# Borda/pyImSegm

Hardware: AMD Instinct MI355X
Metric: Mpixels/s end-to-end SLIC+fts+GC, 2048x2048 RGB; % HBM roofline (higher is better)
Workload: dtype f64; 1 GPU; single 2048x2048 RGB uint8 per GPU, SLIC(sp_size=46, K=2025, 10 sweeps) + colour mean/std/energy + 3-class alpha-expansion GC (gc_regul=2.0, edge=model), pre-fitted GMM, host numpy in -> segm int32 in host numpy (BASELINE configs[1]); bench_config=2, images_per_launch_chain=1, images_in_flight_per_gpu=4, hardware_queues=4, input_memory=pageable numpy, input_ring=default (one rank: measured in round 4), parallelism=images sharded over 1 GPU(s), 4 in flight per GPU (one HIP stream each)

## Files before the change

pyimsegm_amd/_hip.py:

```python
import ctypes as C
import functools
import os
import threading

import numpy as np

_HERE = os.path.dirname(os.path.abspath(__file__))
LIB_PATH = os.environ.get('IMSEGM_HIP_LIBRARY') or os.path.join(_HERE, 'libimsegm_hip.so')

U8, F64, F32 = 0, 1, 2
PROFILE_GROUPS = {
    'slic_assign': 0,
    'slic': 1,
    'connectivity': 2,
    'color_stats': 3,
    'graph': 4,
    'graphcut': 5,
    'gather': 6,
    'slic_preprocess': 7,
    'terms': 8,
    'texture': 9,
}


# ... 1066 lines not shown
        out = np.empty((count.value, 4), dtype=np.float32 if code.value == F32 else np.float64)
        _check(lib.imsegm_volume_get_centroids(self._h, _ptr(out), C.byref(code), C.byref(count)))
        return out

    def label_cc(self):
        n_out = C.c_int(0)
        _check(load_library().imsegm_volume_label_cc(self._h, C.byref(n_out)))
        self.n_labels = n_out.value
        return self.n_labels

    def gray_stats(self, mean=True, energy=True, var=True):
        k = self.n_labels
        m = np.empty(k, dtype=np.float64) if mean else None
        e = np.empty(k, dtype=np.float64) if energy else None
        v = np.empty(k, dtype=np.float64) if var else None
        _check(load_library().imsegm_volume_gray_stats(self._h, _ptr(m), _ptr(e), _ptr(v)))
        return m, e, v

    def graph(self):
        k = self.n_labels
        cap = max(64, 8 * k)
        centres = np.empty((k, 3), dtype=np.float64)
        present = np.empty(k, dtype=np.uint8)
        while True:
            edges = np.empty((cap, 2), dtype=np.int32)
            ne = C.c_int(0)
            _check(load_library().imsegm_volume_graph(self._h, _ptr(edges), cap, C.byref(ne), _ptr(centres),
                                                      _ptr(present)))
            if ne.value <= cap:
                return edges[:ne.value], centres, present.astype(bool)
            cap = ne.value

    def _unsupported(self, *args, **kwargs):
        raise HipError('not available for volumes')

    get_lab = color_stats = run_color = _unsupported

    def lm_prepare(self, sigma=150.):
        taps = gaussian_taps(sigma)
        _check(load_library().imsegm_image2d_lm_prepare(self._h, _ptr(taps), len(taps) - 1, None))
        return self

    def response_stats(self, mul, div, mean=True, energy=True, var=True):
        k = self.n_labels
        m = np.empty(k, dtype=np.float64) if mean else None
        e = np.empty(k, dtype=np.float64) if energy else None
        v = np.empty(k, dtype=np.float64) if var else None
        _check(load_library().imsegm_image2d_response_stats(self._h, float(mul), float(div), _ptr(m), _ptr(e), _ptr(v)))
        return m, e, v

    def response_median(self, mul, div):
        out = np.empty(self.n_labels, dtype=np.float64)
        _check(load_library().imsegm_image2d_response_median(self._h, float(mul), float(div), _ptr(out)))
        return out

    def response_mean_gradient(self, mul, div):
        out = np.empty(self.n_labels, dtype=np.float64)
        _check(load_library().imsegm_image2d_response_mean_gradient(self._h, float(mul), float(div), _ptr(out)))
        return out

    def get_response(self):
        out = np.empty(self.shape, dtype=np.float64)
        _check(load_library().imsegm_image2d_get_response(self._h, _ptr(out)))
        return out


class Batch2D(object):

    def __init__(self, max_images, height, width, ctx=None):
        self.ctx = ctx or default_context()
        self.shape = (int(height), int(width))
        self.max_images = int(max_images)
        self._h = _vp()
        self.n_labels = []
        self.n_images = 0
        _check(load_library().imsegm_batch2d_create(self.ctx._h, self.max_images, self.shape[0], self.shape[1], C.byref(self._h)))
        self.ctx.users += 1

    def close(self):
        if self._h and self.ctx is not None:
            self.ctx.users -= 1
            if self.ctx._h and self.ctx.pid == os.getpid():
                load_library().imsegm_batch2d_destroy(self._h)
        self._h = None

    def __del__(self):
        try:
            self.close()
        except Exception:
            pass

    def run_color(self, images, n_segments, compactness, gmm, pairwise, edge_type='model', feature_flags=(True, True, True),
                  sigma=1., normalize=2, max_iter=10, start_label=0, edge_cost=1., use_graphcut=True, classes=None, to_host=True,
                  pinned=True, out=None):
        images = [np.ascontiguousarray(im) for im in images]
        if not 0 < len(images) <= self.max_images:
            raise ValueError('between 1 and %d images per batch' % self.max_images)
        dtype = images[0].dtype
        if dtype not in _DTYPES or any(im.shape != self.shape + (3, ) or im.dtype != dtype for im in images):
            raise ValueError('expected images of shape %r + (3,) and one dtype of uint8 / float32 / float64' % (self.shape, ))
        code = EDGE_TYPES.get(edge_type)
        if code is None:
            raise ValueError('edge type %r is not evaluated on the device' % (edge_type, ))
        pairwise = np.ascontiguousarray(pairwise, dtype=np.float64)
        nc = gmm.n_classes
        if pairwise.shape != (nc, nc):
            raise ValueError('pairwise cost must be %d x %d' % (nc, nc))
        cl = None if classes is None else np.ascontiguousarray(classes, dtype=np.int32)
        taps = gaussian_taps(sigma)
        r = -1 if taps is None else len(taps) - 1
        n = len(images)
        src = (_vp * n)(*[im.ctypes.data for im in images])
        segm, dst = None, None
        if to_host:
            if out is not None:
                segm = list(out)
                if len(segm) != n or any(a.shape != self.shape or a.dtype != np.int32 or not a.flags['C_CONTIGUOUS'] for a in segm):
                    raise ValueError('out: one C-contiguous int32 array of the image size per image')
            else:
                alloc = pinned_empty if pinned else np.empty
                segm = [alloc(self.shape, np.int32) for _ in range(n)]
            dst = (_vp * n)(*[a.ctypes.data for a in segm])
        mask = (1 if feature_flags[0] else 0) | (2 if feature_flags[1] else 0) | (4 if feature_flags[2] else 0)
        counts = (C.c_int * n)()
        _check(load_library().imsegm_batch2d_run_color(
            self._h, n, src, _DTYPES[dtype], int(normalize), int(n_segments), float(compactness), _ptr(taps), r, int(max_iter),
            int(start_label), mask, C.byref(gmm.params), nc, _ptr(pairwise), code, float(edge_cost), int(bool(use_graphcut)), _ptr(cl),
            dst, counts))
        self.n_labels = list(counts)
        self.n_images = n
        self._feature_columns = 3 * bin(mask).count('1')
        self._uploaded = images
        return segm

    def _device_array(self, image, which):
        ptr = _vp()
        _check(load_library().imsegm_batch2d_device_ptr(self._h, int(image), which, C.byref(ptr)))
        return DeviceArray(ptr.value, self.shape, '<i4', self)

    def segm_device_array(self, image):
        return self._device_array(image, 1)

    def labels_device_array(self, image):
        return self._device_array(image, 0)

    def get_features(self, image):
        ptr = _vp()
        _check(load_library().imsegm_batch2d_device_ptr(self._h, int(image), 2, C.byref(ptr)))
        out = np.empty((self.n_labels[image], self._feature_columns), dtype=np.float64)
        if out.size:
            self.ctx.copy(out.ctypes.data, ptr.value, out.nbytes, synchronize=True)
        return out

    def get_labels(self, image):
        arr = self.labels_device_array(image)
        out = np.empty(self.shape, dtype=np.int32)
        self.ctx.copy(out.ctypes.data, arr.__cuda_array_interface__['data'][0], out.nbytes, synchronize=True)
        return out.astype(np.int64)


class DeviceArray(object):

    def __init__(self, ptr, shape, typestr, owner):
        self.owner = owner
        self.__cuda_array_interface__ = {'shape': tuple(shape), 'typestr': typestr, 'data': (int(ptr), False),
                                         'version': 2, 'strides': None}


def gc_grid_fallbacks():
    return int(load_library().imsegm_debug_gc_grid_fallbacks())


def exclusive_scan(values):
    values = np.ascontiguousarray(values, dtype=np.int32)
    out, total = np.empty_like(values), C.c_int(0)
    _check(load_library().imsegm_debug_exclusive_scan(values.ctypes.data, values.size, out.ctypes.data, C.byref(total)))
    return out, total.value


def slic_sweep_runs():
    a, b = C.c_long(0), C.c_long(0)
    _check(load_library().imsegm_debug_slic_sweep_runs(C.byref(a), C.byref(b)))
    return a.value, b.value


def assign_sweeps_per_launch(max_iter=10):
    persistent, fallback = slic_sweep_runs()
    return max_iter - 1 if (persistent > 0 and fallback == 0) else 1


def _device_array(sess, which, shape, typestr):
    ptr = _vp()
    _check(load_library().imsegm_image2d_device_ptr(sess._h, which, C.byref(ptr)))
    sess.ctx.synchronize()
    return DeviceArray(ptr.value, shape, typestr, sess)


def segm_device_array(sess):
    return _device_array(sess, 1, sess.shape, '<i4')


def cut_general_graph(edges, edge_weights, unary_cost, pairwise_cost, n_iter=-1, algorithm='expansion',
                      return_energy=False, ctx=None):
    if algorithm != 'expansion':
        raise NotImplementedError('only algorithm="expansion" is implemented on the HIP path')
    ctx = ctx or default_context()
    edges = np.ascontiguousarray(np.asarray(edges).reshape(-1, 2), dtype=np.int32)
    ew = np.ascontiguousarray(edge_weights, dtype=np.float64)
    un = np.ascontiguousarray(unary_cost, dtype=np.float64)
    pw = np.ascontiguousarray(pairwise_cost, dtype=np.float64)
    if un.ndim != 2 or pw.shape != (un.shape[1], un.shape[1]) or len(ew) != len(edges):
        raise ValueError('shape mismatch among edges %r, weights %r, unary %r, pairwise %r' %
                         (edges.shape, ew.shape, un.shape, pw.shape))
    labels = np.empty(un.shape[0], dtype=np.int32)
    energy = C.c_int64(0)
    _check(load_library().imsegm_cut_general_graph(ctx._h, _ptr(edges), len(edges), _ptr(ew), _ptr(un), un.shape[0],
                                                   un.shape[1], _ptr(pw), int(n_iter), _ptr(labels), C.byref(energy)))
    return (labels, energy.value) if return_energy else labels


def cut_grid_graph(unary_cost, pairwise_cost, cost_v, cost_h, n_iter=-1, algorithm='expansion', ctx=None):
    unary_cost = np.asarray(unary_cost, dtype=np.float64)
    if unary_cost.ndim != 3:
        raise ValueError('unary_cost must be height x width x labels')
    height, width, n_labels = unary_cost.shape
    cost_v, cost_h = np.asarray(cost_v, dtype=np.float64), np.asarray(cost_h, dtype=np.float64)
    if cost_v.shape != (height - 1, width) or cost_h.shape != (height, width - 1):
        raise ValueError('cost_v / cost_h do not match the grid %d x %d' % (height, width))
    index = np.arange(height * width, dtype=np.int32).reshape(height, width)
    edges = np.concatenate([np.stack([index[:-1].ravel(), index[1:].ravel()], axis=1),
                            np.stack([index[:, :-1].ravel(), index[:, 1:].ravel()], axis=1)], axis=0)
    weights = np.concatenate([cost_v.ravel(), cost_h.ravel()])
    return cut_general_graph(edges, weights, unary_cost.reshape(height * width, n_labels), pairwise_cost, n_iter=n_iter,
                             algorithm=algorithm, ctx=ctx)


def assume_bg_on_boundary(work, strips, bg_label, ctx=None):
    found = C.c_int(0)
    ctx = ctx or default_context()
    _check(load_library().imsegm_assume_bg_on_boundary(ctx._h, _ptr(work), work.shape[0], work.shape[1], _ptr(strips), int(bg_label),
                                                       C.byref(found)))
    return found.value


def label_hist2d(segm, windows, struc_elem, nb_labels, ctx=None):
    ctx = ctx or default_context()
    segm = np.ascontiguousarray(segm, dtype=np.int16)
    selem = np.ascontiguousarray(struc_elem, dtype=np.int16)
    windows = np.ascontiguousarray(windows, dtype=np.int32).reshape(-1, 6)
    out = np.zeros((len(windows), int(nb_labels)), dtype=np.uint32)
    _check(load_library().imsegm_label_hist2d(ctx._h, _ptr(segm), segm.shape[0], segm.shape[1], _ptr(windows), len(windows),
                                              _ptr(selem), selem.shape[0], selem.shape[1], int(nb_labels), _ptr(out)))
    return out


BOUNDARY_THICK, BOUNDARY_CONTOUR, BOUNDARY_CONTOUR_BORDER = 0, 1, 2


def boundary_mask(labels, mode, label=0, ctx=None):
    ctx = ctx or default_context()
    out = np.empty(labels.shape, dtype=np.uint8)
    _check(load_library().imsegm_boundary_mask(ctx._h, _ptr(labels), labels.shape[0], labels.shape[1], int(mode), int(label), _ptr(out)))
    return out


def distance_map(labels, mode, label=0, ctx=None):
    ctx = ctx or default_context()
    out = np.empty(labels.shape, dtype=np.float64)
    _check(load_library().imsegm_distance_map(ctx._h, _ptr(labels), labels.shape[0], labels.shape[1], int(mode), int(label), _ptr(out)))
    return out


def _boundary_distances(call, shape):
    capacity = int(shape[0]) * int(shape[1])
    points, dist, count = np.empty((capacity, 2), dtype=np.int32), np.empty(capacity, dtype=np.float64), C.c_int(0)
    _check(call(_ptr(points), _ptr(dist), capacity, C.byref(count)))
    return points[:count.value], dist[:count.value].copy()


def boundary_distances(segm_ref, segm, ctx=None):
    ctx = ctx or default_context()
    lib = load_library()
    return _boundary_distances(lambda *out: lib.imsegm_boundary_distances(ctx._h, _ptr(segm_ref), _ptr(segm), segm.shape[0],
                                                                          segm.shape[1], *out), segm.shape)


def labels_overlap(seg1, seg2, n_labels1, n_labels2, ctx=None):
    ctx = ctx or default_context()
    out = np.empty((int(n_labels1), int(n_labels2)), dtype=np.int64)
    _check(load_library().imsegm_labels_overlap(ctx._h, _ptr(seg1), _ptr(seg2), seg1.size, int(n_labels1), int(n_labels2), _ptr(out)))
    return out


def ellipse_ransac(point_offsets, points, params, success, trial_egg, points_all, point_value, residual_threshold,
                   with_residuals=False, ctx=None):
    ctx = ctx or default_context()
    point_offsets = np.ascontiguousarray(point_offsets, dtype=np.int32).ravel()
    points = np.ascontiguousarray(points, dtype=np.float64).reshape(-1, 2)
    params = np.ascontiguousarray(params, dtype=np.float64).reshape(-1, 5)
    success = np.ascontiguousarray(success, dtype=np.uint8).ravel()
    trial_egg = np.ascontiguousarray(trial_egg, dtype=np.int32).ravel()
    points_all = np.ascontiguousarray(points_all, dtype=np.float64).reshape(-1, 2)
    point_value = np.ascontiguousarray(point_value, dtype=np.float64).ravel()
    n_eggs, n_trials = len(point_offsets) - 1, len(params)
    if len(success) != n_trials or len(trial_egg) != n_trials or len(point_value) != len(points_all):
        raise ValueError('ellipse_ransac: one success flag and one egg per trial, one value per centre')
# ... 180 lines not shown
```

pyimsegm_amd/csrc/batch.hip:

```cpp
#include "backhalf.h"

#include <string>

struct imsegm_batch2d {
    imsegm_ctx *ctx = nullptr;
    int B = 0, H = 0, W = 0;
    size_t n = 0;
    DevBuf arena;
    size_t slice = 0;
    std::vector<unsigned char> key;
    int *fail_host = nullptr;
    void *pinned = nullptr;
    size_t pinned_cap = 0;
    int last_n = 0;
    std::vector<int> n_labels;
};

namespace {

using namespace imsegm;

inline size_t al256(size_t v) { return (v + 255) & ~(size_t)255; }

struct Layout {
    size_t img, lab, nearest, labels, conn_i32, conn_i32_bytes, conn_u8, small, cent, tiles, feat, featK, seg, segm_out, total;
    ParamBlock par;
    TermsScratch scr;
    size_t d_edges, d_as, d_at, d_ar, d_ea, d_deg, d_dlow, d_es, d_wp, d_cacc, d_bitmap, d_cent, d_present;
    int Kb, Ecap;
};

Layout make_layout(int H, int W, size_t elem, int K_grid, size_t n_tiles, long min_size, int C, int F, int Fm, int n_in)
{
    Layout L;
    memset(&L, 0, sizeof(L));
    const size_t n = (size_t)H * W;
    L.Kb = (int)std::min<size_t>(n / (size_t)std::max<long>(min_size, 1) + 2, n + 2);
    L.Ecap = 3 * L.Kb + 64;
    size_t o = 0;
    auto take = [&](size_t bytes) { size_t at = o; o += al256(bytes); return at; };
    L.small = take(4096);
    L.img = take(n * 3 * elem + 64);
    L.lab = take(3 * n * sizeof(double));
    L.nearest = take(n * 4);
    L.labels = take(n * 4);
    L.conn_i32_bytes = conn_i32_bytes(n, H, W);
    L.conn_i32 = take(L.conn_i32_bytes);
    L.conn_u8 = take(2 * n + 64);
    L.cent = take(slic_cent_bytes(K_grid));
    L.tiles = take(slic_tiles_bytes(n_tiles, n));
    const size_t Kb = (size_t)L.Kb, E = (size_t)L.Ecap, words = (size_t)cdiv(L.Kb, 32);
    L.feat = take(stats_scratch_bytes(Kb));
    L.featK = take(Kb * (size_t)std::max(F, 1) * 8 + 64);
    L.segm_out = take(n * 4);
    L.par = param_block(C, Fm, 0, n_in);
    L.scr = terms_scratch(L.par, L.Kb, C, F, L.Ecap, false, n_in ? Fm : 0);
    size_t q = L.scr.end;
    auto sub = [&](size_t bytes) { size_t at = q; q += al64(bytes); return at; };
    L.d_edges = sub(E * 8);
    L.d_as = sub((Kb + 1) * 4);
    L.d_at = sub(E * 8);
    L.d_ar = sub(E * 8);
    L.d_ea = sub(E * 8);
    L.d_deg = sub(Kb * 4);
    L.d_dlow = sub(Kb * 4);
    L.d_es = sub(Kb * 4);
    L.d_wp = sub(Kb * words * 4);
    L.d_cacc = sub(Kb * 4 * 8);
    L.d_bitmap = sub(Kb * words * 4);
    L.d_cent = sub(Kb * 3 * 8);
    L.d_present = sub(Kb);
    L.seg = take(q + 256);
    L.total = al256(o);
    return L;
}

int batch_pinned(imsegm_batch2d *bt, size_t bytes)
{
    if (bytes <= bt->pinned_cap) return 0;
    if (bt->pinned) (void)hipHostFree(bt->pinned);
    bt->pinned = nullptr;
    bt->pinned_cap = 0;
    HIP_TRY(hipHostMalloc(&bt->pinned, bytes + 4096, hipHostMallocDefault));
    bt->pinned_cap = bytes + 4096;
    return 0;
}

}

extern "C" {

int imsegm_batch2d_create(imsegm_ctx *ctx, int max_images, int height, int width, imsegm_batch2d **batch_out)
{
    if (bind(ctx)) return -1;
    if (!batch_out || max_images < 1 || max_images > 1024 || height <= 0 || width <= 0 || (long)height * width > 0x3fffffffL) {
        set_error("batch2d: 1..1024 images of a valid size");
        return -1;
    }
    imsegm_batch2d *bt = new imsegm_batch2d();
    bt->ctx = ctx;
    bt->B = max_images;
    bt->H = height;
    bt->W = width;
    bt->n = (size_t)height * width;
    bt->n_labels.assign(max_images, 0);
    *batch_out = bt;
    return 0;
}

void imsegm_batch2d_destroy(imsegm_batch2d *bt)
{
    if (!bt) return;
    (void)hipSetDevice(bt->ctx->device);
    (void)hipStreamSynchronize(bt->ctx->stream);
    bt->arena.release();
    if (bt->fail_host) (void)hipHostFree(bt->fail_host);
    if (bt->pinned) (void)hipHostFree(bt->pinned);
    delete bt;
}

int imsegm_batch2d_device_ptr(imsegm_batch2d *bt, int image, int which, void **ptr_out)
{
    if (!bt || bind(bt->ctx)) return -1;
    if (!ptr_out || image < 0 || image >= bt->last_n || bt->key.size() != sizeof(Layout)) {
        set_error("batch2d_device_ptr: no such image in the last batch");
        return -1;
    }
    Layout L;
    memcpy(&L, bt->key.data(), sizeof(L));
    unsigned char *base = bt->arena.as<unsigned char>() + (size_t)image * bt->slice;
    if (which == 0) *ptr_out = base + L.labels;
    else if (which == 1) *ptr_out = base + L.segm_out;
    else if (which == 2) *ptr_out = base + L.featK;
    else {
        set_error("batch2d_device_ptr: which = 0 (label map), 1 (segmentation) or 2 (feature table)");
        return -1;
    }
    return 0;
}

int imsegm_batch2d_run_color(imsegm_batch2d *bt, int n_images, const void *const *host_pixels, int dtype, int minmax_normalize,
                             int n_segments, double compactness, const double *taps, int radius, int max_iter, int start_label,
                             int feature_mask, const imsegm_gmm *gmm, int n_classes, const double *pairwise, int edge_type,
                             double edge_cost, int use_graphcut, const int32_t *classes_lut, int32_t *const *segm_out,
                             int *n_labels_out)
{
    if (!bt || bind(bt->ctx)) return -1;
    imsegm_ctx *ctx = bt->ctx;
    hipStream_t st = ctx->stream;
    const int H = bt->H, W = bt->W, C = n_classes;
    const size_t n = bt->n;
    if (n_images < 1 || n_images > bt->B || !host_pixels) {
        set_error("batch2d_run_color: between 1 and the batch's capacity of images");
        return -1;
    }
    const size_t es = dtype == IMSEGM_U8 ? 1 : dtype == IMSEGM_F32 ? 4 : dtype == IMSEGM_F64 ? 8 : 0;
    if (!es) {
        set_error("unsupported dtype");
        return -1;
    }
    if (!(compactness > 0) || n_segments < 1 || max_iter < 1 || (start_label != 0 && start_label != 1)) {
        set_error("slic: n_segments, compactness and max_iter must be positive, start_label 0 or 1");
        return -1;
    }
    if (feature_mask < 1 || feature_mask > 7 || !gmm || C < 1 || C > 16 || !pairwise) {
        set_error("batch2d_run_color: colour features (mask 1..7), a device class model, 1..16 classes and a pairwise matrix are required");
        return -1;
    }
    BackHalf bh;
    if (decode_edge_type(edge_type, &bh.edge_code, &bh.spatial_norm)) return -1;
    const int F = color_feature_columns(feature_mask);
    if (check_gmm(gmm, F, C)) return -1;
    if (check_pairwise(pairwise, C)) return -1;
    Taps tz, ty, tx;
    if (fill_taps(tz, taps, radius) || fill_taps(ty, taps, radius) || fill_taps(tx, taps, radius)) return -1;
    if (radius > 8 || knobs().pre_3pass) {
        set_error("batch2d_run_color: blur radius above 8 (sigma > 2) takes the single-image path");
        return -1;
    }

    SlicState s;
    SlicGeometry geo;
    if (slic_geometry(H, W, n_segments, compactness, minmax_normalize, 0, 0, s, geo)) return -1;
    const int K = geo.K;
    const double segment_size = (double)n / (double)K;
    const long min_size = (long)(0.5 * segment_size), max_size = (long)(3.0 * segment_size);
    if (min_size < 1) {
        set_error("batch2d_run_color: superpixels of under two pixels take the single-image path");
        return -1;
    }
    const Layout L = make_layout(H, W, es, K, geo.n_tiles, min_size, C, F, gmm->n_features, gmm->n_inputs);
    const size_t slice = L.total;
    const size_t stage_row = al256(std::max<size_t>(L.par.bytes, 256));
    const size_t arena_bytes = slice * bt->B + stage_row * bt->B + 4096;
    const bool same = bt->key.size() == sizeof(L) && !memcmp(bt->key.data(), &L, sizeof(L)) && bt->slice == slice && bt->arena.cap >= arena_bytes;
    if (!same) {
        HIP_TRY(hipStreamSynchronize(st));
        if (bt->arena.ensure(arena_bytes)) return -1;
        HIP_TRY(hipMemsetAsync(bt->arena.p, 0, bt->arena.cap, st));
        bt->slice = slice;
        bt->key.assign(reinterpret_cast<const unsigned char *>(&L), reinterpret_cast<const unsigned char *>(&L) + sizeof(L));
    }
    if (!bt->fail_host) HIP_TRY(hipHostMalloc((void **)&bt->fail_host, 64, hipHostMallocDefault));
    unsigned char *base = bt->arena.as<unsigned char>();
    unsigned char *stage_dev = base + slice * bt->B;
    ZBatch zb;
    zb.nz = n_images;
    zb.zs = slice;
    bt->last_n = n_images;

    bool all_pinned = true;
    for (int b = 0; b < n_images; ++b) {
        if (!host_pixels[b]) {
            set_error("batch2d_run_color: null image");
            return -1;
        }
        HIP_TRY(hipMemcpyAsync(base + (size_t)b * slice + L.img, host_pixels[b], n * 3 * es, hipMemcpyHostToDevice, st));
        all_pinned = all_pinned && is_pinned(host_pixels[b]);
    }
    if (!all_pinned) HIP_TRY(hipStreamSynchronize(st));

    unsigned long long *keys = reinterpret_cast<unsigned long long *>(base + L.small);
    double *minmax = reinterpret_cast<double *>(keys + 2);
    double *premax = minmax + 2;
    double *lab = reinterpret_cast<double *>(base + L.lab);
    int32_t *nearest = reinterpret_cast<int32_t *>(base + L.nearest), *labels = reinterpret_cast<int32_t *>(base + L.labels);
    const int sp_all = ctx->begin(PG_SLIC);
    const int sp_pre = ctx->begin(PG_PRE);
    if (launch_minmax(base + L.img, dtype, n * 3, keys, minmax, st, premax, zb)) return -1;
    if (launch_preprocess_color2d(base + L.img, dtype, H, W, minmax_normalize, minmax, tz, ty, tx, 1.0 / compactness, lab, nullptr, premax,
                                  st, true, zb))
        return -1;
    ctx->end(sp_pre);
    slic_place_state(s, geo, base + L.cent, base + L.tiles, premax, bt->fail_host);
    const ProfHook hook = ctx->hook();
    bool fused_update = false;
    if (launch_slic_iterations(s, lab, nullptr, nearest, max_iter, 0, hook, st, &fused_update, zb)) return -1;

    ConnWork w = conn_work_from(reinterpret_cast<int32_t *>(base + L.conn_i32), L.conn_i32_bytes, base + L.conn_u8, n);
    std::vector<int> &nl = bt->n_labels;
    for (int attempt = 0; attempt < 2; ++attempt) {
        if (attempt == 1) {
            slic_sweep_note_fallback();
            SlicState plain = s;
            plain.done = nullptr;
            if (launch_slic_iterations(plain, lab, nullptr, nearest, max_iter, 0, hook, st, nullptr, zb)) return -1;
        }
        const int spc = ctx->begin(PG_CONN);
        if (launch_enforce_connectivity_batch(nearest, H, W, min_size, max_size, start_label, w, labels, nl.data(), st, zb,
                                              reinterpret_cast<int32_t *>(stage_dev)))
            return -1;
        ctx->end(spc);
        if (!fused_update || *bt->fail_host == 0) break;
        fused_update = false;
    }
    for (int b = 0; b < n_images; ++b) {
        if (nl[b] >= 0) continue;
        unsigned char *sb = base + (size_t)b * slice;
        ConnWork wb = conn_work_from(reinterpret_cast<int32_t *>(sb + L.conn_i32), L.conn_i32_bytes, sb + L.conn_u8, n);
        int got = 0;
        if (launch_enforce_connectivity(reinterpret_cast<int32_t *>(sb + L.nearest), 1, H, W, min_size, max_size, start_label, wb,
                                        reinterpret_cast<int32_t *>(sb + L.labels), &got, st))
            return -1;
        nl[b] = got;
    }
    ctx->end(sp_all);
    int K_cap = 1;
    for (int b = 0; b < n_images; ++b) {
        if (nl[b] > L.Kb) {
            set_error("batch2d_run_color: more labels than the bound the buffers were sized for");
            return -1;
        }
        K_cap = std::max(K_cap, nl[b]);
        if (n_labels_out) n_labels_out[b] = nl[b];
    }
    const int words = cdiv(K_cap, 32);
    const int Ecap = std::min(L.Ecap, 3 * K_cap + 64);

    {
        const StatsScratch ss = stats_scratch_at(base + L.feat, L.Kb);
        const double *mm_dev = nullptr;
        if (dtype != IMSEGM_U8) {
            if (launch_minmax(base + L.img, dtype, n * 3, keys, minmax, st, nullptr, zb)) return -1;
            mm_dev = minmax;
        }
        const int sps = ctx->begin(PG_STATS);
        if (launch_color_stats(base + L.img, dtype, labels, H, W, K_cap, 255.0, (feature_mask & 2) != 0, ss.acc, ss.mean, ss.energy, ss.var,
                               ss.mean32, st, 0, 0, 1.0, 1.0, -1, nullptr, zb, mm_dev))
// ... 59 lines not shown
```

pyimsegm_amd/csrc/slic_pre.hip:

```cpp
#include "slic.h"
#include <hip/hip_ext.h>
#include <atomic>
#include <cstdio>


namespace imsegm {

__device__ __forceinline__ unsigned long long f64_key(double x)
{
    long long b = __double_as_longlong(x);
    return b < 0 ? ~(unsigned long long)b : ((unsigned long long)b | 0x8000000000000000ULL);
}
__host__ __device__ __forceinline__ double key_f64(unsigned long long k)
{
    unsigned long long b = (k & 0x8000000000000000ULL) ? (k & 0x7fffffffffffffffULL) : ~k;
    union { unsigned long long u; double d; } cv;
    cv.u = b;
    return cv.d;
}

__device__ __forceinline__ void block_minmax_commit(double mn, double mx, unsigned long long *keys, double *out2, double *also_zero)
{
    __shared__ double smn[4], smx[4];
    mn = wave_min_f64(mn);
// ... 103 lines not shown
    if (tz.r < 0) return v;
    double tmp = v * tz.w[0];
    for (int j = tz.r; j >= 1; --j) tmp += (v + v) * tz.w[j];
    return tmp;
}

template <int MAXR>
__device__ __forceinline__ double zblur_point_unrolled(double v, const Taps &tz)
{
    if (tz.r < 0) return v;
    double tmp = v * tz.w[0];
    const double vv = v + v;
#pragma unroll
    for (int j = MAXR; j >= 1; --j)
        if (j <= tz.r) tmp += vv * tz.w[j];
    return tmp;
}

__global__ void __launch_bounds__(256)
k_pre_lab_u8(const uint8_t *__restrict__ img, int n, int normalize, const double *__restrict__ minmax,
             Taps tz, double *__restrict__ out)
{
    __shared__ double lut[256];
    {
        int v = threadIdx.x;
        double x;
        const bool norm = normalize == 1 || (normalize == 2 && (minmax[0] != 0.0 || minmax[1] != 1.0));
        if (norm) {
            double vmin = minmax[0], range = minmax[1] - minmax[0];
            x = (double)(uint8_t)(v - (int)vmin) / range;
        } else {
            x = (double)v * (1.0 / 255);
        }
        lut[v] = (x > 0.04045) ? det_pow24((x + 0.055) / 1.055) : x / 12.92;
    }
    __syncthreads();
    int p = blockIdx.x * blockDim.x + threadIdx.x;
    if (p >= n) return;
    double lin0 = lut[img[3 * (size_t)p + 0]], lin1 = lut[img[3 * (size_t)p + 1]], lin2 = lut[img[3 * (size_t)p + 2]];
    double X = lin0 * 0.412453 + lin1 * 0.357580 + lin2 * 0.180423;
    double Y = lin0 * 0.212671 + lin1 * 0.715160 + lin2 * 0.072169;
    double Z = lin0 * 0.019334 + lin1 * 0.119193 + lin2 * 0.950227;
    double f[3] = { X / 0.95047, Y / 1.0, Z / 1.08883 };
#pragma unroll
    for (int c = 0; c < 3; ++c) {
        double t = f[c];
        f[c] = (t > 0.008856) ? det_cbrt(t) : 7.787 * t + 16.0 / 116.0;
    }
    double L = (116.0 * f[1]) - 16.0;
    double A = 500.0 * (f[0] - f[1]);
    double B = 200.0 * (f[1] - f[2]);
    out[p] = zblur_point(L, tz);
    out[(size_t)n + p] = zblur_point(A, tz);
    out[2 * (size_t)n + p] = zblur_point(B, tz);
}

template <typename T>
__global__ void __launch_bounds__(256)
k_pre_lab_f(const T *__restrict__ img, int n, int normalize, const double *__restrict__ minmax, Taps tz,
            double *__restrict__ out)
{
    int p = blockIdx.x * blockDim.x + threadIdx.x;
    if (p >= n) return;
    double rgb[3];
    const bool norm = normalize == 1 || (normalize == 2 && (minmax[0] != 0.0 || minmax[1] != 1.0));
#pragma unroll
    for (int c = 0; c < 3; ++c) {
        double v = (double)img[3 * (size_t)p + c];
        if (norm) v = (v - minmax[0]) / (minmax[1] - minmax[0]);
        rgb[c] = v;
    }
    double L, A, B;
    rgb2lab_px(rgb[0], rgb[1], rgb[2], L, A, B);
    out[p] = zblur_point(L, tz);
    out[(size_t)n + p] = zblur_point(A, tz);
    out[2 * (size_t)n + p] = zblur_point(B, tz);
}

__device__ __forceinline__ void block_absmax_to(double v, double *out)
{
    __shared__ unsigned long long wave_max[16];
    unsigned long long b = (unsigned long long)__double_as_longlong(v);
#pragma unroll
    for (int off = 32; off > 0; off >>= 1) {
        unsigned long long o = __shfl_xor(b, off, 64);
        b = o > b ? o : b;
    }
    const int wave = threadIdx.x >> 6, nw = (blockDim.x + 63) >> 6;
    if ((threadIdx.x & 63) == 0) wave_max[wave] = b;
    __syncthreads();
    if (threadIdx.x == 0) {
        for (int i = 1; i < nw; ++i) b = wave_max[i] > b ? wave_max[i] : b;
        if (b) atomicMax(reinterpret_cast<unsigned long long *>(out), b);
    }
}

__global__ void __launch_bounds__(256) k_absmax_f64(const double *__restrict__ src, size_t n, double *out)
{
    double m = 0.0;
    for (size_t i = (size_t)blockIdx.x * 256 + threadIdx.x; i < n; i += (size_t)gridDim.x * 256) m = fmax(m, fabs(src[i]));
    block_absmax_to(m, out);
}

int launch_absmax_f64(const double *src, size_t n, double *out_dev, hipStream_t st)
{
    HIP_TRY(hipMemsetAsync(out_dev, 0, sizeof(double), st));
    int grid = (int)std::min<size_t>(2048, (n + 256 * 8 - 1) / (256 * 8));
    hipLaunchKernelGGL(k_absmax_f64, grid < 1 ? 1 : grid, 256, 0, st, src, n, out_dev);
    HIP_TRY(hipGetLastError());
    return 0;
}

__device__ __forceinline__ int reflect_idx(int i, int n)
{
    if ((unsigned)i < (unsigned)n) return i;
    if (n == 1) return 0;
    int p = 2 * n;
    i %= p;
    if (i < 0) i += p;
    if (i >= n) i = p - 1 - i;
    return i;
}

template <int AXIS>
__global__ void __launch_bounds__(256)
k_blur_axis(const double *__restrict__ src, double *__restrict__ dst, int H, int W, Taps t, double ratio, int scale)
{
    int x = blockIdx.x * 64 + (threadIdx.x & 63);
    int y = blockIdx.y * 4 + (threadIdx.x >> 6);
    int plane = blockIdx.z;
    if (x >= W || y >= H) return;
    const double *s = src + (size_t)plane * H * W;
    double v;
    if (t.r < 0) {
        v = s[(size_t)y * W + x];
    } else {
        v = s[(size_t)y * W + x] * t.w[0];
        for (int j = t.r; j >= 1; --j) {
            double a, b;
            if (AXIS == 0) {
                a = s[(size_t)reflect_idx(y - j, H) * W + x];
                b = s[(size_t)reflect_idx(y + j, H) * W + x];
            } else {
                a = s[(size_t)y * W + reflect_idx(x - j, W)];
                b = s[(size_t)y * W + reflect_idx(x + j, W)];
            }
            v += (a + b) * t.w[j];
        }
    }
    if (scale) v = v * ratio;
    dst[(size_t)plane * H * W + (size_t)y * W + x] = v;
}

constexpr int PF_TX = 64, PF_TY = 16, PF_MAXR = 8, PF_THREADS = 512;
static_assert(PF_THREADS % PF_TX == 0 && PF_TY % (PF_THREADS / PF_TX) == 0, "x pass: whole rows per pass");

template <typename T>
__global__ void __launch_bounds__(PF_THREADS)
k_pre_fused(const T *__restrict__ img, int H, int W, int normalize, const double *__restrict__ minmax, Taps tz, Taps ty,
            Taps tx, double ratio, double *__restrict__ out, double *premax, size_t zs)
{
    ZSHIFT(img, zs); ZSHIFT(minmax, zs); ZSHIFT(out, zs); ZSHIFT(premax, zs);
    double vmax = 0.0;
    extern __shared__ double pf_sm[];
    __shared__ double lut[256];
    const int tid = threadIdx.x;
    const int ry = ty.r < 0 ? 0 : ty.r, rx = tx.r < 0 ? 0 : tx.r;
    const int tw = PF_TX + 2 * rx, th = PF_TY + 2 * ry;
    const unsigned int tw_magic = (unsigned int)((0x100000000ull + tw - 1) / tw);
    double *L1 = pf_sm;
    double *L2 = pf_sm + (size_t)3 * th * tw;
    const bool norm = normalize == 1 || (normalize == 2 && (minmax[0] != 0.0 || minmax[1] != 1.0));
    if (sizeof(T) == 1) {
        if (tid < 256) {
            const int v = tid;
            double x;
            if (norm) {
                double vmin = minmax[0], range = minmax[1] - minmax[0];
                x = (double)(uint8_t)(v - (int)vmin) / range;
            } else {
                x = (double)v * (1.0 / 255);
            }
            lut[v] = (x > 0.04045) ? det_pow24((x + 0.055) / 1.055) : x / 12.92;
        }
        __syncthreads();
    }
    const int x0 = blockIdx.x * PF_TX, y0 = blockIdx.y * PF_TY;
    const size_t plane = (size_t)H * W;
    for (int i = tid; i < th * tw; i += PF_THREADS) {
        const int ly = (int)__umulhi((unsigned int)i, tw_magic), lx = i - ly * tw;
        const int gy = reflect_idx(y0 + ly - ry, H), gx = reflect_idx(x0 + lx - rx, W);
        const size_t p = (size_t)gy * W + gx;
        double L, A, B;
        if (sizeof(T) == 1) {
            double lin0 = lut[(int)img[3 * p + 0]], lin1 = lut[(int)img[3 * p + 1]], lin2 = lut[(int)img[3 * p + 2]];
            double X = lin0 * 0.412453 + lin1 * 0.357580 + lin2 * 0.180423;
            double Y = lin0 * 0.212671 + lin1 * 0.715160 + lin2 * 0.072169;
            double Z = lin0 * 0.019334 + lin1 * 0.119193 + lin2 * 0.950227;
            double f[3] = { DIV_CONST_IN_RANGE(X, 0.95047), Y, DIV_CONST_IN_RANGE(Z, 1.08883) };
#pragma unroll
            for (int c = 0; c < 3; ++c) {
                double t = f[c];
                f[c] = (t > 0.008856) ? det_cbrt(t) : 7.787 * t + 16.0 / 116.0;
            }
            L = (116.0 * f[1]) - 16.0;
            A = 500.0 * (f[0] - f[1]);
            B = 200.0 * (f[1] - f[2]);
        } else {
            double rgb[3];
#pragma unroll
            for (int c = 0; c < 3; ++c) {
                double v = (double)img[3 * p + c];
                if (norm) v = (v - minmax[0]) / (minmax[1] - minmax[0]);
                rgb[c] = v;
            }
            rgb2lab_px(rgb[0], rgb[1], rgb[2], L, A, B);
        }
        L1[i] = zblur_point_unrolled<PF_MAXR>(L, tz);
        L1[th * tw + i] = zblur_point_unrolled<PF_MAXR>(A, tz);
        L1[2 * th * tw + i] = zblur_point_unrolled<PF_MAXR>(B, tz);
    }
    __syncthreads();
    const int ox = tid % PF_TX, oy0 = tid / PF_TX;
    for (int c = 0; c < 3; ++c) {
        const double *s1 = L1 + (size_t)c * th * tw;
        for (int i = tid; i < PF_TY * tw; i += PF_THREADS) {
            const int oy = (int)__umulhi((unsigned int)i, tw_magic), lx = i - oy * tw;
            const double *col = s1 + (oy + ry) * tw + lx;
            double v;
            if (ty.r < 0) {
                v = col[0];
            } else {
                v = col[0] * ty.w[0];
#pragma unroll
                for (int j = PF_MAXR; j >= 1; --j)
                    if (j <= ty.r) v += (col[-j * tw] + col[j * tw]) * ty.w[j];
            }
            L2[i] = v;
        }
        __syncthreads();
#pragma unroll
        for (int q = 0; q < PF_TY / (PF_THREADS / PF_TX); ++q) {
            const int oy = oy0 + (PF_THREADS / PF_TX) * q;
            const double *row = L2 + oy * tw + ox + rx;
            double v;
            if (tx.r < 0) {
                v = row[0];
            } else {
                v = row[0] * tx.w[0];
#pragma unroll
                for (int j = PF_MAXR; j >= 1; --j)
                    if (j <= tx.r) v += (row[-j] + row[j]) * tx.w[j];
            }
            v = v * ratio;
            const int gy = y0 + oy, gx = x0 + ox;
            if (gy < H && gx < W) {
                out[(size_t)c * plane + (size_t)gy * W + gx] = v;
                vmax = fmax(vmax, fabs(v));
            }
        }
        __syncthreads();
    }
    block_absmax_to(vmax, premax);
}

int launch_preprocess_color2d(const void *img, int dtype, int H, int W, int normalize, const double *minmax_dev,
                              const Taps &tz, const Taps &ty, const Taps &tx, double ratio, double *bufA,
                              double *bufB, double *premax_dev, hipStream_t st, bool premax_zeroed, ZBatch zb)
{
    int n = H * W;
    int grid = cdiv(n, 256);
    if (tz.r <= PF_MAXR && ty.r <= PF_MAXR && tx.r <= PF_MAXR && !knobs().pre_3pass) {
        const int ry = ty.r < 0 ? 0 : ty.r, rx = tx.r < 0 ? 0 : tx.r;
        const size_t lds = ((size_t)3 * (PF_TY + 2 * ry) + PF_TY) * (PF_TX + 2 * rx) * sizeof(double);
        const void *fn = dtype == DT_U8 ? (const void *)k_pre_fused<uint8_t>
                       : dtype == DT_F32 ? (const void *)k_pre_fused<float> : (const void *)k_pre_fused<double>;
        static size_t lds_set[IMSEGM_MAX_DEVICES][3];
        int dev = 0;
        HIP_TRY(hipGetDevice(&dev));
        if (dev < 0 || dev >= IMSEGM_MAX_DEVICES || lds_set[dev][dtype] < lds) {
            HIP_TRY(hipFuncSetAttribute(fn, hipFuncAttributeMaxDynamicSharedMemorySize, (int)lds));
            if (dev >= 0 && dev < IMSEGM_MAX_DEVICES) lds_set[dev][dtype] = lds;
        }
        dim3 gf(cdiv(W, PF_TX), cdiv(H, PF_TY), zb.nz);
        if (!premax_zeroed) {
            if (zb.nz > 1) {
                set_error("preprocess: a batch needs its premax words zeroed by the caller");
                return -1;
            }
            HIP_TRY(hipMemsetAsync(premax_dev, 0, sizeof(double), st));
        }
        if (dtype == DT_U8)
            hipLaunchKernelGGL(k_pre_fused<uint8_t>, gf, PF_THREADS, lds, st, (const uint8_t *)img, H, W, normalize, minmax_dev, tz, ty, tx,
                               ratio, bufA, premax_dev, zb.zs);
        else if (dtype == DT_F32)
            hipLaunchKernelGGL(k_pre_fused<float>, gf, PF_THREADS, lds, st, (const float *)img, H, W, normalize, minmax_dev, tz, ty, tx,
                               ratio, bufA, premax_dev, zb.zs);
        else
            hipLaunchKernelGGL(k_pre_fused<double>, gf, PF_THREADS, lds, st, (const double *)img, H, W, normalize, minmax_dev, tz, ty, tx,
                               ratio, bufA, premax_dev, zb.zs);
        HIP_TRY(hipGetLastError());
        return 0;
    }
    if (zb.nz > 1) {
        set_error("preprocess: the three-pass path (blur radius > 8) does not take a batch");
        return -1;
    }
    if (dtype == DT_U8)
        hipLaunchKernelGGL(k_pre_lab_u8, grid, 256, 0, st, (const uint8_t *)img, n, normalize, minmax_dev, tz, bufA);
    else if (dtype == DT_F32)
        hipLaunchKernelGGL(k_pre_lab_f<float>, grid, 256, 0, st, (const float *)img, n, normalize, minmax_dev, tz, bufA);
    else
        hipLaunchKernelGGL(k_pre_lab_f<double>, grid, 256, 0, st, (const double *)img, n, normalize, minmax_dev, tz, bufA);
    dim3 g(cdiv(W, 64), cdiv(H, 4), 3);
    hipLaunchKernelGGL(k_blur_axis<0>, g, 256, 0, st, bufA, bufB, H, W, ty, ratio, 0);
    hipLaunchKernelGGL(k_blur_axis<1>, g, 256, 0, st, bufB, bufA, H, W, tx, ratio, 1);
    HIP_TRY(hipGetLastError());
    return launch_absmax_f64(bufA, (size_t)3 * n, premax_dev, st);
}

}
```

Baseline: 5574 Mpixels/s.

## Add radius-4 specialised fused preprocess kernel with register-blocked y-blur

Adds a specialised fused Lab-conversion plus separable blur kernel for the common case where all blur radii equal 4. It uses 1024-thread workgroups on a 64x32 tile, does the y-blur in place with per-thread register windows of 8 outputs so no second LDS buffer is needed, and loads the three uint8 channels with one 4-byte load. The generic kernel is kept for other radii, and debug accessors for the Lab planes and pre-processing scalars are exposed. The aim is to cut LDS traffic and halo overhead in preprocessing, at the cost of register pressure and extra code paths.

```diff
diff --git a/pyimsegm_amd/_hip.py b/pyimsegm_amd/_hip.py
--- a/pyimsegm_amd/_hip.py
+++ b/pyimsegm_amd/_hip.py
@@ -1242,6 +1242,19 @@
             self.ctx.copy(out.ctypes.data, ptr.value, out.nbytes, synchronize=True)
         return out
 
+    def _get_f64(self, image, which, shape):
+        ptr = _vp()
+        _check(load_library().imsegm_batch2d_device_ptr(self._h, int(image), which, C.byref(ptr)))
+        out = np.empty(shape, dtype=np.float64)
+        self.ctx.copy(out.ctypes.data, ptr.value, out.nbytes, synchronize=True)
+        return out
+
+    def get_lab(self, image):
+        return self._get_f64(image, 3, (3, ) + self.shape)
+
+    def get_pre_scalars(self, image):
+        return tuple(float(v) for v in self._get_f64(image, 4, (3, )))
+
     def get_labels(self, image):
         arr = self.labels_device_array(image)
         out = np.empty(self.shape, dtype=np.int32)
diff --git a/pyimsegm_amd/csrc/batch.hip b/pyimsegm_amd/csrc/batch.hip
--- a/pyimsegm_amd/csrc/batch.hip
+++ b/pyimsegm_amd/csrc/batch.hip
@@ -132,8 +132,10 @@
     if (which == 0) *ptr_out = base + L.labels;
     else if (which == 1) *ptr_out = base + L.segm_out;
     else if (which == 2) *ptr_out = base + L.featK;
+    else if (which == 3) *ptr_out = base + L.lab;
+    else if (which == 4) *ptr_out = base + L.small + 2 * sizeof(unsigned long long);
     else {
-        set_error("batch2d_device_ptr: which = 0 (label map), 1 (segmentation) or 2 (feature table)");
+        set_error("batch2d_device_ptr: which = 0 (label map), 1 (segmentation), 2 (feature table), 3 (pre-processed planes) or 4 (min, max, premax)");
         return -1;
     }
     return 0;
diff --git a/pyimsegm_amd/csrc/slic_pre.hip b/pyimsegm_amd/csrc/slic_pre.hip
--- a/pyimsegm_amd/csrc/slic_pre.hip
+++ b/pyimsegm_amd/csrc/slic_pre.hip
@@ -279,13 +279,200 @@
     dst[(size_t)plane * H * W + (size_t)y * W + x] = v;
 }
 
-constexpr int PF_TX = 64, PF_TY = 16, PF_MAXR = 8, PF_THREADS = 512;
-static_assert(PF_THREADS % PF_TX == 0 && PF_TY % (PF_THREADS / PF_TX) == 0, "x pass: whole rows per pass");
+constexpr int PF_TX = 64, PF_MAXR = 8, PF_THREADS = 512;
+
+__device__ __forceinline__ void pf_fill_lut(double *lut, bool norm, const double *__restrict__ minmax)
+{
+    if (threadIdx.x < 256) {
+        const int v = threadIdx.x;
+        double x;
+        if (norm) {
+            double vmin = minmax[0], range = minmax[1] - minmax[0];
+            x = (double)(uint8_t)(v - (int)vmin) / range;
+        } else {
+            x = (double)v * (1.0 / 255);
+        }
+        lut[v] = (x > 0.04045) ? det_pow24((x + 0.055) / 1.055) : x / 12.92;
+    }
+}
+
+__device__ __forceinline__ uint32_t pf_load_u8(const uint8_t *__restrict__ img, size_t p, size_t n_pixels)
+{
+    uint32_t w;
+    if (p + 1 < n_pixels)
+        __builtin_memcpy(&w, img + 3 * p, 4);
+    else
+        w = (uint32_t)img[3 * p] | ((uint32_t)img[3 * p + 1] << 8) | ((uint32_t)img[3 * p + 2] << 16);
+    return w;
+}
+
+template <int ZR>
+__device__ __forceinline__ double pf_ztap(double v, const Taps &tz)
+{
+    if constexpr (ZR < 0) {
+        return zblur_point_unrolled<PF_MAXR>(v, tz);
+    } else {
+        double tmp = v * tz.w[0];
+        const double vv = v + v;
+#pragma unroll
+        for (int j = ZR; j >= 1; --j) tmp += vv * tz.w[j];
+        return tmp;
+    }
+}
+
+template <int ZR>
+__device__ __forceinline__ void pf_lab_u8(uint32_t w, const double *lut, const Taps &tz, double &L, double &A, double &B)
+{
+    double lin0 = lut[w & 0xffu], lin1 = lut[(w >> 8) & 0xffu], lin2 = lut[(w >> 16) & 0xffu];
+    double X = lin0 * 0.412453 + lin1 * 0.357580 + lin2 * 0.180423;
+    double Y = lin0 * 0.212671 + lin1 * 0.715160 + lin2 * 0.072169;
+    double Z = lin0 * 0.019334 + lin1 * 0.119193 + lin2 * 0.950227;
+    double f[3] = { DIV_CONST_IN_RANGE(X, 0.95047), Y, DIV_CONST_IN_RANGE(Z, 1.08883) };
+#pragma unroll
+    for (int c = 0; c < 3; ++c) {
+        double t = f[c];
+        f[c] = (t > 0.008856) ? det_cbrt(t) : 7.787 * t + 16.0 / 116.0;
+    }
+    L = pf_ztap<ZR>((116.0 * f[1]) - 16.0, tz);
+    A = pf_ztap<ZR>(500.0 * (f[0] - f[1]), tz);
+    B = pf_ztap<ZR>(200.0 * (f[1] - f[2]), tz);
+}
+
+template <int ZR, typename T>
+__device__ __forceinline__ void pf_lab_f(const T *__restrict__ img, size_t p, bool norm, const double *__restrict__ minmax, const Taps &tz,
+                                         double &L, double &A, double &B)
+{
+    double rgb[3];
+#pragma unroll
+    for (int c = 0; c < 3; ++c) {
+        double v = (double)img[3 * p + c];
+        if (norm) v = (v - minmax[0]) / (minmax[1] - minmax[0]);
+        rgb[c] = v;
+    }
+    rgb2lab_px(rgb[0], rgb[1], rgb[2], L, A, B);
+    L = pf_ztap<ZR>(L, tz);
+    A = pf_ztap<ZR>(A, tz);
+    B = pf_ztap<ZR>(B, tz);
+}
+
+constexpr int P4_R = 4, P4_TY = 32, P4_RUN = 8, P4_THREADS = 1024;
+constexpr int P4_TW = PF_TX + 2 * P4_R, P4_TH = P4_TY + 2 * P4_R, P4_PLANE = P4_TH * P4_TW;
+constexpr int P4_NCONV = (P4_PLANE + P4_THREADS - 1) / P4_THREADS;
+constexpr int P4_G = P4_TY / P4_RUN, P4_NY = 3 * P4_G * P4_TW;
+constexpr int P4_YITEMS = (P4_NY + P4_THREADS - 1) / P4_THREADS;
+constexpr int P4_ROWS = P4_THREADS / PF_TX;
+constexpr size_t P4_LDS = (size_t)3 * P4_PLANE * sizeof(double);
+static_assert(P4_TY % P4_RUN == 0 && P4_TY % P4_ROWS == 0 && P4_THREADS % PF_TX == 0, "whole windows, whole rows per round");
+static_assert(2 * (P4_LDS + 256 * sizeof(double) + 16 * sizeof(unsigned long long)) <= 160 * 1024, "two workgroups a CU");
+
+template <typename T>
+__global__ void __launch_bounds__(P4_THREADS, 8)
+k_pre_fused(const T *__restrict__ img, int H, int W, int normalize, const double *__restrict__ minmax, Taps tz, Taps ty,
+            Taps tx, double ratio, double *__restrict__ out, double *premax, size_t zs)
+{
+    ZSHIFT(img, zs); ZSHIFT(minmax, zs); ZSHIFT(out, zs); ZSHIFT(premax, zs);
+    extern __shared__ double pf_sm[];
+    __shared__ double lut[256];
+    const int tid = threadIdx.x;
+    const int x0 = blockIdx.x * PF_TX, y0 = blockIdx.y * P4_TY;
+    const size_t plane = (size_t)H * W;
+    const bool norm = normalize == 1 || (normalize == 2 && (minmax[0] != 0.0 || minmax[1] != 1.0));
+    if constexpr (sizeof(T) == 1) {
+        pf_fill_lut(lut, norm, minmax);
+        __syncthreads();
+        uint32_t px[P4_NCONV];
+#pragma unroll
+        for (int k = 0; k < P4_NCONV; ++k) {
+            const int i = tid + k * P4_THREADS;
+            if (i < P4_PLANE) {
+                const int ly = i / P4_TW, lx = i - ly * P4_TW;
+                const int gy = reflect_idx(y0 + ly - P4_R, H), gx = reflect_idx(x0 + lx - P4_R, W);
+                px[k] = pf_load_u8(img, (size_t)gy * W + gx, plane);
+            }
+        }
+#pragma unroll
+        for (int k = 0; k < P4_NCONV; ++k) {
+            const int i = tid + k * P4_THREADS;
+            if (i < P4_PLANE) {
+                double L, A, B;
+                pf_lab_u8<P4_R>(px[k], lut, tz, L, A, B);
+                pf_sm[i] = L;
+                pf_sm[P4_PLANE + i] = A;
+                pf_sm[2 * P4_PLANE + i] = B;
+            }
+        }
+    } else {
+        for (int i = tid; i < P4_PLANE; i += P4_THREADS) {
+            const int ly = i / P4_TW, lx = i - ly * P4_TW;
+            const int gy = reflect_idx(y0 + ly - P4_R, H), gx = reflect_idx(x0 + lx - P4_R, W);
+            double L, A, B;
+            pf_lab_f<P4_R>(img, (size_t)gy * W + gx, norm, minmax, tz, L, A, B);
+            pf_sm[i] = L;
+            pf_sm[P4_PLANE + i] = A;
+            pf_sm[2 * P4_PLANE + i] = B;
+        }
+    }
+    __syncthreads();
+    double yo[P4_YITEMS][P4_RUN];
+#pragma unroll
+    for (int k = 0; k < P4_YITEMS; ++k) {
+        const int item = tid + k * P4_THREADS;
+        if (item < P4_NY) {
+            const int cg = item / P4_TW, lx = item - cg * P4_TW;
+            const double *col = pf_sm + ((cg / P4_G) * P4_TH + (cg % P4_G) * P4_RUN) * P4_TW + lx;
+            double win[P4_RUN + 2 * P4_R];
+#pragma unroll
+            for (int m = 0; m < P4_RUN + 2 * P4_R; ++m) win[m] = col[m * P4_TW];
+#pragma unroll
+            for (int q = 0; q < P4_RUN; ++q) {
+                double v = win[q + P4_R] * ty.w[0];
+#pragma unroll
+                for (int j = P4_R; j >= 1; --j) v += (win[q + P4_R - j] + win[q + P4_R + j]) * ty.w[j];
+                yo[k][q] = v;
+            }
+        }
+    }
+    __syncthreads();
+#pragma unroll
+    for (int k = 0; k < P4_YITEMS; ++k) {
+        const int item = tid + k * P4_THREADS;
+        if (item < P4_NY) {
+            const int cg = item / P4_TW, lx = item - cg * P4_TW;
+            double *col = pf_sm + ((cg / P4_G) * P4_TH + (cg % P4_G) * P4_RUN) * P4_TW + lx;
+#pragma unroll
+            for (int q = 0; q < P4_RUN; ++q) col[q * P4_TW] = yo[k][q];
+        }
+    }
+    __syncthreads();
+    double vmax = 0.0;
+    const int ox = tid % PF_TX, oy0 = tid / PF_TX;
+    const int gx = x0 + ox;
+    for (int c = 0; c < 3; ++c) {
+#pragma unroll
+        for (int q = 0; q < P4_TY / P4_ROWS; ++q) {
+            const int oy = oy0 + P4_ROWS * q;
+            const double *row = pf_sm + (c * P4_TH + oy) * P4_TW + ox + P4_R;
+            double v = row[0] * tx.w[0];
+#pragma unroll
+            for (int j = P4_R; j >= 1; --j) v += (row[-j] + row[j]) * tx.w[j];
+            v = v * ratio;
+            const int gy = y0 + oy;
+            if (gy < H && gx < W) {
+                out[(size_t)c * plane + (size_t)gy * W + gx] = v;
+                vmax = fmax(vmax, fabs(v));
+            }
+        }
+    }
+    block_absmax_to(vmax, premax);
+}
+
+constexpr int PF_TY = 16;
+static_assert(PF_TY % (PF_THREADS / PF_TX) == 0, "x pass: whole rows per pass");
 
 template <typename T>
 __global__ void __launch_bounds__(PF_THREADS)
-k_pre_fused(const T *__restrict__ img, int H, int W, int normalize, const double *__restrict__ minmax, Taps tz, Taps ty,
-            Taps tx, double ratio, double *__restrict__ out, double *premax, size_t zs)
+k_pre_fused_any(const T *__restrict__ img, int H, int W, int normalize, const double *__restrict__ minmax, Taps tz, Taps ty,
+                Taps tx, double ratio, double *__restrict__ out, double *premax, size_t zs)
 {
     ZSHIFT(img, zs); ZSHIFT(minmax, zs); ZSHIFT(out, zs); ZSHIFT(premax, zs);
     double vmax = 0.0;
@@ -299,17 +486,7 @@
     double *L2 = pf_sm + (size_t)3 * th * tw;
     const bool norm = normalize == 1 || (normalize == 2 && (minmax[0] != 0.0 || minmax[1] != 1.0));
     if (sizeof(T) == 1) {
-        if (tid < 256) {
-            const int v = tid;
-            double x;
-            if (norm) {
-                double vmin = minmax[0], range = minmax[1] - minmax[0];
-                x = (double)(uint8_t)(v - (int)vmin) / range;
-            } else {
-                x = (double)v * (1.0 / 255);
-            }
-            lut[v] = (x > 0.04045) ? det_pow24((x + 0.055) / 1.055) : x / 12.92;
-        }
+        pf_fill_lut(lut, norm, minmax);
         __syncthreads();
     }
     const int x0 = blockIdx.x * PF_TX, y0 = blockIdx.y * PF_TY;
@@ -319,33 +496,13 @@
         const int gy = reflect_idx(y0 + ly - ry, H), gx = reflect_idx(x0 + lx - rx, W);
         const size_t p = (size_t)gy * W + gx;
         double L, A, B;
-        if (sizeof(T) == 1) {
-            double lin0 = lut[(int)img[3 * p + 0]], lin1 = lut[(int)img[3 * p + 1]], lin2 = lut[(int)img[3 * p + 2]];
-            double X = lin0 * 0.412453 + lin1 * 0.357580 + lin2 * 0.180423;
-            double Y = lin0 * 0.212671 + lin1 * 0.715160 + lin2 * 0.072169;
-            double Z = lin0 * 0.019334 + lin1 * 0.119193 + lin2 * 0.950227;
-            double f[3] = { DIV_CONST_IN_RANGE(X, 0.95047), Y, DIV_CONST_IN_RANGE(Z, 1.08883) };
-#pragma unroll
-            for (int c = 0; c < 3; ++c) {
-                double t = f[c];
-                f[c] = (t > 0.008856) ? det_cbrt(t) : 7.787 * t + 16.0 / 116.0;
-            }
-            L = (116.0 * f[1]) - 16.0;
-            A = 500.0 * (f[0] - f[1]);
-            B = 200.0 * (f[1] - f[2]);
-        } else {
-            double rgb[3];
-#pragma unroll
-            for (int c = 0; c < 3; ++c) {
-                double v = (double)img[3 * p + c];
-                if (norm) v = (v - minmax[0]) / (minmax[1] - minmax[0]);
-                rgb[c] = v;
-            }
-            rgb2lab_px(rgb[0], rgb[1], rgb[2], L, A, B);
-        }
-        L1[i] = zblur_point_unrolled<PF_MAXR>(L, tz);
-        L1[th * tw + i] = zblur_point_unrolled<PF_MAXR>(A, tz);
-        L1[2 * th * tw + i] = zblur_point_unrolled<PF_MAXR>(B, tz);
+        if constexpr (sizeof(T) == 1)
+            pf_lab_u8<-1>(pf_load_u8(img, p, plane), lut, tz, L, A, B);
+        else
+            pf_lab_f<-1>(img, p, norm, minmax, tz, L, A, B);
+        L1[i] = L;
+        L1[th * tw + i] = A;
+        L1[2 * th * tw + i] = B;
     }
     __syncthreads();
     const int ox = tid % PF_TX, oy0 = tid / PF_TX;
@@ -391,6 +548,27 @@
     block_absmax_to(vmax, premax);
 }
 
+template <typename T>
+static int launch_pre_fused(const T *img, int H, int W, int normalize, const double *minmax_dev, const Taps &tz, const Taps &ty,
+                            const Taps &tx, double ratio, double *out, double *premax_dev, hipStream_t st, ZBatch zb, int dtype)
+{
+    const bool r4 = tz.r == P4_R && ty.r == P4_R && tx.r == P4_R;
+    const int ry = ty.r < 0 ? 0 : ty.r, rx = tx.r < 0 ? 0 : tx.r;
+    const size_t lds = r4 ? P4_LDS : ((size_t)3 * (PF_TY + 2 * ry) + PF_TY) * (PF_TX + 2 * rx) * sizeof(double);
+    const auto fn = r4 ? k_pre_fused<T> : k_pre_fused_any<T>;
+    static size_t lds_set[IMSEGM_MAX_DEVICES][2][3];
+    int dev = 0;
+    HIP_TRY(hipGetDevice(&dev));
+    if (dev < 0 || dev >= IMSEGM_MAX_DEVICES || lds_set[dev][r4][dtype] < lds) {
+        HIP_TRY(hipFuncSetAttribute((const void *)fn, hipFuncAttributeMaxDynamicSharedMemorySize, (int)lds));
+        if (dev >= 0 && dev < IMSEGM_MAX_DEVICES) lds_set[dev][r4][dtype] = lds;
+    }
+    const dim3 grid(cdiv(W, PF_TX), cdiv(H, r4 ? P4_TY : PF_TY), zb.nz);
+    hipLaunchKernelGGL(fn, grid, r4 ? P4_THREADS : PF_THREADS, lds, st, img, H, W, normalize, minmax_dev, tz, ty, tx, ratio, out, premax_dev, zb.zs);
+    HIP_TRY(hipGetLastError());
+    return 0;
+}
+
 int launch_preprocess_color2d(const void *img, int dtype, int H, int W, int normalize, const double *minmax_dev,
                               const Taps &tz, const Taps &ty, const Taps &tx, double ratio, double *bufA,
                               double *bufB, double *premax_dev, hipStream_t st, bool premax_zeroed, ZBatch zb)
@@ -398,18 +576,6 @@
     int n = H * W;
     int grid = cdiv(n, 256);
     if (tz.r <= PF_MAXR && ty.r <= PF_MAXR && tx.r <= PF_MAXR && !knobs().pre_3pass) {
-        const int ry = ty.r < 0 ? 0 : ty.r, rx = tx.r < 0 ? 0 : tx.r;
-        const size_t lds = ((size_t)3 * (PF_TY + 2 * ry) + PF_TY) * (PF_TX + 2 * rx) * sizeof(double);
-        const void *fn = dtype == DT_U8 ? (const void *)k_pre_fused<uint8_t>
-                       : dtype == DT_F32 ? (const void *)k_pre_fused<float> : (const void *)k_pre_fused<double>;
-        static size_t lds_set[IMSEGM_MAX_DEVICES][3];
-        int dev = 0;
-        HIP_TRY(hipGetDevice(&dev));
-        if (dev < 0 || dev >= IMSEGM_MAX_DEVICES || lds_set[dev][dtype] < lds) {
-            HIP_TRY(hipFuncSetAttribute(fn, hipFuncAttributeMaxDynamicSharedMemorySize, (int)lds));
-            if (dev >= 0 && dev < IMSEGM_MAX_DEVICES) lds_set[dev][dtype] = lds;
-        }
-        dim3 gf(cdiv(W, PF_TX), cdiv(H, PF_TY), zb.nz);
         if (!premax_zeroed) {
             if (zb.nz > 1) {
                 set_error("preprocess: a batch needs its premax words zeroed by the caller");
@@ -418,16 +584,10 @@
             HIP_TRY(hipMemsetAsync(premax_dev, 0, sizeof(double), st));
         }
         if (dtype == DT_U8)
-            hipLaunchKernelGGL(k_pre_fused<uint8_t>, gf, PF_THREADS, lds, st, (const uint8_t *)img, H, W, normalize, minmax_dev, tz, ty, tx,
-                               ratio, bufA, premax_dev, zb.zs);
-        else if (dtype == DT_F32)
-            hipLaunchKernelGGL(k_pre_fused<float>, gf, PF_THREADS, lds, st, (const float *)img, H, W, normalize, minmax_dev, tz, ty, tx,
-                               ratio, bufA, premax_dev, zb.zs);
-        else
-            hipLaunchKernelGGL(k_pre_fused<double>, gf, PF_THREADS, lds, st, (const double *)img, H, W, normalize, minmax_dev, tz, ty, tx,
-                               ratio, bufA, premax_dev, zb.zs);
-        HIP_TRY(hipGetLastError());
-        return 0;
+            return launch_pre_fused((const uint8_t *)img, H, W, normalize, minmax_dev, tz, ty, tx, ratio, bufA, premax_dev, st, zb, dtype);
+        if (dtype == DT_F32)
+            return launch_pre_fused((const float *)img, H, W, normalize, minmax_dev, tz, ty, tx, ratio, bufA, premax_dev, st, zb, dtype);
+        return launch_pre_fused((const double *)img, H, W, normalize, minmax_dev, tz, ty, tx, ratio, bufA, premax_dev, st, zb, dtype);
     }
     if (zb.nz > 1) {
         set_error("preprocess: the three-pass path (blur radius > 8) does not take a batch");
```

Measured after the change: 5869 Mpixels/s (median of 6 runs). 5.3% higher.
